# eniac/Reef

Measured on AMD Instinct MI355X. Metric: msm_scalar_point_pairs_per_sec, higher is better.
Workload: dtype u32

## Files before the change

include/reef_msm.h:

```cpp
#ifndef REEF_MSM_H
#define REEF_MSM_H
#define REEF_ABI_VERSION 7

#include <stdbool.h>
#include <stddef.h>
#include <stdint.h>

#ifdef __cplusplus
extern "C" {
#endif

typedef struct { uint64_t l[4]; } reef_fe;
typedef struct { reef_fe x, y; } reef_affine;
typedef struct { reef_fe x, y, z; } reef_jacobian;

enum { REEF_PALLAS = 0, REEF_VESTA = 1 };
enum { REEF_HOST = 0, REEF_DEVICE = 1 };

typedef enum {
    REEF_OK = 0,
    REEF_ERR_ARG = 1,
    REEF_ERR_HIP = 2,
    REEF_ERR_NO_GPU = 3,
    REEF_ERR_OOM = 4
// ... 165 lines not shown
uint32_t reef_abi_version(void);
enum { REEF_WARM_NONE = 0, REEF_WARM_NOW = 1, REEF_WARM_BACKGROUND = 2 };
typedef struct {
    int32_t hw_queues;
    uint32_t warm;
    uint32_t reserved[6];
} reef_runtime_opts;
typedef struct {
    int32_t hw_queues_env;
    int32_t hw_queues_set_by_library;
    uint32_t abi_version;
    uint32_t warm;
} reef_runtime_info;
reef_status reef_runtime_init(const reef_runtime_opts *opts , reef_runtime_info *info );

reef_status reef_msm_ctx_set_window_split(reef_msm_ctx *ctx, uint32_t rank, uint32_t world);
reef_status reef_msm_ctx_enable_timing(reef_msm_ctx *ctx, int on);
reef_status reef_msm_ctx_last_timing(reef_msm_ctx *ctx, float *total_ms, float *accumulate_ms);
reef_status reef_msm_ctx_timing_stats(reef_msm_ctx *ctx, int reset, uint64_t *calls, double *total_ms,
                                      double *accumulate_ms);
reef_status reef_msm_ctx_sum_points(reef_msm_ctx *ctx, const reef_jacobian *in, size_t n, reef_jacobian *out);
reef_status reef_msm_ctx_plan(reef_msm_ctx *ctx, uint32_t *c, uint32_t *windows, uint32_t *groups,
                              uint32_t *tables);

reef_status reef_msm_plan_for(size_t n, uint32_t window_bits, uint32_t bucket_groups, uint32_t *c,
                              uint32_t *windows, uint32_t *groups, uint32_t *tables);

reef_status reef_test_field_op(int field, int op, const reef_fe *a, const reef_fe *b, reef_fe *out, size_t n);
reef_status reef_test_ec_op(int curve, int op, const reef_affine *p, const reef_affine *q, const reef_fe *k,
                            reef_jacobian *out, size_t n);
reef_status reef_bench_fmul(int field, uint32_t iters, double *products_per_s);

typedef struct reef_msm_group reef_msm_group;
enum { REEF_SPLIT_WINDOWS = 0, REEF_SPLIT_POINTS = 1 };
enum { REEF_EXCHANGE_DEFAULT = 0, REEF_EXCHANGE_PEER = 1, REEF_EXCHANGE_HOST = 2, REEF_EXCHANGE_RCCL = 3 };
enum { REEF_SCALARS_EACH = 0, REEF_SCALARS_FANOUT = 1 };
typedef struct {
    uint32_t split;
    uint32_t exchange;
    uint32_t scalars;
    uint32_t reserved[5];
} reef_msm_group_opts;
typedef struct {
    uint32_t members;
    uint32_t distinct_devices;
    uint32_t split, exchange;
// ... 28 lines not shown
```

reef_amd/_ffi.py:

```python
from __future__ import annotations

import ctypes
import os
import subprocess
from ctypes import POINTER, c_bool, c_char_p, c_double, c_float, c_int, c_int32, c_size_t, c_uint8, c_uint32, c_uint64, c_void_p

_HERE = os.path.dirname(os.path.abspath(__file__))
CSRC = os.path.join(_HERE, "csrc")
if os.environ.get("REEF_MSM_HW_QUEUES", "") != "0":
    os.environ.setdefault("GPU_MAX_HW_QUEUES", os.environ.get("REEF_MSM_HW_QUEUES") or "8")
LIB_PATH = os.environ.get("REEF_MSM_LIB") or os.path.join(_HERE, "_lib", "libreef_msm.so")
EXPERIMENT_LIB_PATH = os.path.join(_HERE, "_lib", "libreef_msm_exp.so")
HEADER = os.path.join(os.path.dirname(_HERE), "include", "reef_msm.h")

REEF_HOST, REEF_DEVICE = 0, 1
PALLAS, VESTA = 0, 1
STATUS_NAMES = {0: "REEF_OK", 1: "REEF_ERR_ARG", 2: "REEF_ERR_HIP", 3: "REEF_ERR_NO_GPU", 4: "REEF_ERR_OOM"}


class ReefError(RuntimeError):
    def __init__(self, status: int, message: str):
        super().__init__(f"{STATUS_NAMES.get(status, status)}: {message}")
        self.status = status

# ... 79 lines not shown
        "reef_gen_bases": (c_int, [c_int, c_uint64, c_uint64, c_size_t, vp, c_int]),
        "reef_gen_scalars": (c_int, [c_int, c_uint64, c_int, c_uint64, c_size_t, c_bool, vp, c_int]),
        "reef_device_count": (c_int, []),
        "reef_set_device": (c_int, [c_int]),
        "reef_get_device": (c_int, [POINTER(c_int)]),
        "reef_device_sync": (c_int, []),
        "reef_device_alloc": (vp, [c_size_t]),
        "reef_device_free": (None, [vp]),
        "reef_memcpy": (c_int, [vp, vp, c_size_t, c_int, c_int]),
        "reef_last_error": (c_char_p, []),
        "reef_version": (c_char_p, []),
        "reef_abi_version": (c_uint32, []),
        "reef_key_cache_info": (None, [POINTER(KeyCacheStats)]),
        "reef_key_cache_clear": (None, []),
        "reef_key_cache_wait": (None, []),
        "reef_key_cache_timing_get": (None, [POINTER(KeyCacheTiming), c_int]),
        "reef_runtime_init": (c_int, [POINTER(RuntimeOpts), POINTER(RuntimeInfo)]),
        "reef_msm_ctx_last_timing": (c_int, [vp, POINTER(c_float), POINTER(c_float)]),
        "reef_msm_ctx_enable_timing": (c_int, [vp, c_int]),
        "reef_msm_ctx_set_window_split": (c_int, [vp, c_uint32, c_uint32]),
        "reef_msm_ctx_timing_stats": (c_int, [vp, c_int, POINTER(c_uint64), POINTER(c_double), POINTER(c_double)]),
        "reef_msm_ctx_sum_points": (c_int, [vp, vp, c_size_t, vp]),
        "reef_msm_ctx_plan": (c_int, [vp, POINTER(c_uint32), POINTER(c_uint32), POINTER(c_uint32), POINTER(c_uint32)]),
        "reef_msm_ctx_byte_tables": (c_int, [vp]),
        "reef_msm_plan_for": (c_int, [c_size_t, c_uint32, c_uint32, POINTER(c_uint32), POINTER(c_uint32), POINTER(c_uint32),
                                      POINTER(c_uint32)]),
        "reef_msm_group_create": (c_int, [POINTER(vp), c_int, vp, c_size_t, c_int, POINTER(MsmOpts), POINTER(c_int), c_size_t, POINTER(GroupOpts)]),
        "reef_msm_group_destroy": (None, [vp]),
        "reef_msm_group_info_get": (c_int, [vp, POINTER(GroupInfo)]),
        "reef_msm_group_enable_timing": (c_int, [vp, c_int]),
        "reef_msm_group_last_timing": (c_int, [vp, POINTER(GroupTiming)]),
        "reef_msm_group_msm": (c_int, [vp, vp, c_size_t, c_int, c_bool, vp]),
        "reef_msm_group_rows": (c_int, [vp, vp, c_size_t, c_size_t, c_int, c_bool, c_uint32, vp, vp, vp]),
        "reef_msm_group_rows_symbols": (c_int, [vp, vp, c_size_t, c_size_t, c_int, c_uint32, vp, vp, c_bool, vp]),
        "reef_msm_folded": (c_int, [vp, vp, c_size_t, c_size_t, c_int, c_bool, vp, vp, c_size_t, vp, c_int]),
        "reef_sc_create": (c_int, [POINTER(vp), c_int, c_size_t]),
        "reef_sc_destroy": (None, [vp]),
        "reef_sc_set_table": (c_int, [vp, c_int, vp, c_size_t, c_int]),
        "reef_sc_gen_eq_table": (c_int, [vp, vp, vp, c_size_t, vp, c_size_t]),
        "reef_sc_round_coeffs": (c_int, [vp, c_size_t, vp]),
        "reef_sc_fold": (c_int, [vp, c_size_t, vp]),
        "reef_sc_fold_and_next_coeffs": (c_int, [vp, c_size_t, vp, vp]),
        "reef_sc_read": (c_int, [vp, c_int, c_size_t, vp]),
        "reef_sc_reset_table": (c_int, [vp]),
        "reef_sc_sync": (c_int, [vp]),
        "reef_nifs_create": (c_int, [POINTER(vp), c_int, c_size_t, c_size_t, c_size_t, c_int]),
# ... 95 lines not shown
```

reef_amd/csrc/api.cpp:

```cpp
#include <stdarg.h>
#include <stdio.h>
#include <string>
#include <vector>
#include <new>
#include <exception>
#include <stdlib.h>
#include <string.h>

#include <atomic>
#include <chrono>
#include <condition_variable>
#include <deque>
#include <memory>
#include <mutex>
#include <thread>
#include <type_traits>

#include "common.h"
#include "keccak.h"

namespace reef {

static thread_local char g_err[512] = "";

// ... 264 lines not shown
}
void reef_msm_ctx_destroy(reef_msm_ctx *ctx) { destroy_handle(ctx, &CurveVTable::ctx_destroy); }
reef_status reef_msm_ctx_sync(reef_msm_ctx *ctx) {
    return dispatch<CurveVTable>(ctx, [&](auto *v, void *impl) { return v->ctx_sync(impl); });
}
void *reef_msm_ctx_stream(reef_msm_ctx *ctx) { return ctx ? table<CurveVTable>(ctx->curve)->ctx_stream(ctx->impl) : nullptr; }
reef_status reef_msm_ctx_last_timing(reef_msm_ctx *ctx, float *total_ms, float *accumulate_ms) {
    return dispatch<CurveVTable>(ctx, [&](auto *v, void *impl) { return v->ctx_timing(impl, total_ms, accumulate_ms); });
}
reef_status reef_msm_ctx_set_window_split(reef_msm_ctx *ctx, uint32_t rank, uint32_t world) {
    return dispatch<CurveVTable>(ctx, [&](auto *v, void *impl) { return v->ctx_window_split(impl, rank, world); });
}
reef_status reef_msm_ctx_enable_timing(reef_msm_ctx *ctx, int on) {
    return dispatch<CurveVTable>(ctx, [&](auto *v, void *impl) { return v->ctx_enable_timing(impl, on); });
}
reef_status reef_msm_ctx_timing_stats(reef_msm_ctx *ctx, int reset, uint64_t *calls, double *total_ms, double *accumulate_ms) {
    return dispatch<CurveVTable>(ctx, [&](auto *v, void *impl) { return v->ctx_timing_stats(impl, reset, calls, total_ms, accumulate_ms); });
}
reef_status reef_msm_ctx_sum_points(reef_msm_ctx *ctx, const reef_jacobian *in, size_t n, reef_jacobian *out) {
    return dispatch<CurveVTable>(ctx, [&](auto *v, void *impl) { return v->ctx_sum_points(impl, in, n, out); });
}
reef_status reef_msm_ctx_plan(reef_msm_ctx *ctx, uint32_t *c, uint32_t *windows, uint32_t *groups, uint32_t *tables) {
    return dispatch<CurveVTable>(ctx, [&](auto *v, void *impl) { return v->ctx_plan(impl, c, windows, groups, tables); });
}

reef_status reef_msm(reef_msm_ctx *ctx, const reef_fe *scalars, size_t n, int scalars_loc, bool is_mont, reef_jacobian *out,
                     int out_loc) {
    return dispatch<CurveVTable>(ctx, [&](auto *v, void *impl) { return v->msm(impl, scalars, n, scalars_loc, is_mont, out, out_loc); });
}
reef_status reef_msm_rows(reef_msm_ctx *ctx, const reef_fe *scalars, size_t rows, size_t row_len, int scalars_loc, bool is_mont,
                          uint32_t max_scalar_bits, const reef_fe *blinds, const reef_affine *h, reef_jacobian *out, int out_loc) {
    return dispatch<CurveVTable>(ctx, [&](auto *v, void *impl) { return v->msm_rows(impl, scalars, rows, row_len, scalars_loc, is_mont, max_scalar_bits, blinds, h, out, out_loc); });
}

reef_status reef_msm_multi(size_t count, reef_msm_ctx *const *ctxs, const reef_fe *const *scalars, const size_t *n, int scalars_loc, bool is_mont,
                           reef_jacobian *out) {
    if (count == 0) return REEF_OK;
    if (!ctxs || !scalars || !n || !out || count > 64) { set_error("reef_msm_multi: null argument or more than 64 MSMs"); return REEF_ERR_ARG; }
    for (size_t i = 0; i < count; ++i) {
        if (!ctxs[i]) { set_error("null argument"); return REEF_ERR_ARG; }
        for (size_t j = 0; j < i; ++j)
            if (ctxs[j] == ctxs[i]) { set_error("reef_msm_multi: contexts must be distinct (clone a key that is used twice)"); return REEF_ERR_ARG; }
    }
    static thread_local struct Landing {
        reef_jacobian *p = nullptr;
        ~Landing() { if (p && !g_process_exiting.load()) (void)hipHostFree(p); }
// ... 945 lines not shown
```

reef_amd/csrc/common.h:

```cpp
#pragma once
#include <algorithm>
#include <atomic>
#include <mutex>
#include <thread>
#include <stdio.h>
#include <stdlib.h>
#include <vector>
#include <hip/hip_runtime.h>
#include <stddef.h>
#include <stdint.h>

#include "../../include/reef_msm.h"

namespace reef {

void set_error(const char *fmt, ...) __attribute__((format(printf, 1, 2)));

#define REEF_HIP_TRY(expr)                                                                          \
    do {                                                                                            \
        hipError_t e_ = (expr);                                                                     \
        if (e_ != hipSuccess) {                                                                     \
            ::reef::set_error("%s: %s (%s:%d)", #expr, hipGetErrorString(e_), __FILE__, __LINE__);  \
            return e_ == hipErrorOutOfMemory ? REEF_ERR_OOM : REEF_ERR_HIP;                         \
        }                                                                                           \
// ... 294 lines not shown
struct MerkleSlice {
    uint64_t index_base = 0;
    uint32_t levels = 0;
    const reef_fe *nodes_in = nullptr;
    size_t nodes_n = 0;
    reef_fe *const *level_out = nullptr;
    reef_fe *top_out = nullptr;
};

struct CurveVTable {
    reef_status (*ctx_create)(void **impl, const reef_affine *bases, size_t n, int loc, const reef_msm_opts *opts);
    reef_status (*ctx_rekey)(void *impl, const reef_affine *bases, size_t n, int loc);
    reef_status (*ctx_clone)(void **impl, void *src);
    reef_status (*ctx_attach)(void *impl, void *src_impl);
    void (*ctx_destroy)(void *impl);
    reef_status (*ctx_sync)(void *impl);
    void *(*ctx_stream)(void *impl);
    reef_status (*ctx_timing)(void *impl, float *total_ms, float *acc_ms);
    reef_status (*ctx_enable_timing)(void *impl, int on);
    reef_status (*ctx_window_split)(void *impl, uint32_t rank, uint32_t world);
    reef_status (*ctx_timing_stats)(void *impl, int reset, uint64_t *calls, double *total_ms, double *acc_ms);
    reef_status (*ctx_sum_points)(void *impl, const reef_jacobian *in, size_t n, reef_jacobian *out);
    reef_status (*ctx_plan)(void *impl, uint32_t *c, uint32_t *w, uint32_t *g, uint32_t *t);
    int (*ctx_byte_tables)(void *impl);
    reef_status (*msm)(void *impl, const reef_fe *scalars, size_t n, int loc, bool is_mont, reef_jacobian *out, int out_loc);
    reef_status (*msm_rows)(void *impl, const reef_fe *scalars, size_t rows, size_t row_len, int loc, bool is_mont,
                            uint32_t max_bits, const reef_fe *blinds, const reef_affine *h, reef_jacobian *out, int out_loc);
    reef_status (*msm_rows_symbols)(void *impl, const uint8_t *symbols, size_t rows, size_t row_len, int loc, uint32_t bits,
                                    const reef_fe *blinds, const reef_affine *h, bool blinds_are_mont, reef_jacobian *out, int out_loc);
    reef_status (*ipa_cross)(void *impl, const reef_fe *a, size_t n_k, int loc, bool is_mont, const reef_fe *w1s, const reef_fe *w2s, size_t k,
                             reef_jacobian *out_l, reef_jacobian *out_r);
    reef_status (*msm_folded)(void *impl, const reef_fe *v, size_t len, size_t off, int loc, bool is_mont, const reef_fe *w1s, const reef_fe *w2s,
                              size_t k, reef_jacobian *out, int out_loc);
    reef_status (*fold)(const reef_affine *gens, size_t half, int loc, const reef_fe *w1, const reef_fe *w2, reef_affine *out);
    reef_status (*normalize)(const reef_jacobian *in, size_t n, int loc, reef_affine *out_aff, uint8_t *out_comp);
    reef_status (*sum_points)(const reef_jacobian *in, size_t n, int loc, reef_jacobian *out);
    reef_status (*gen_bases)(uint64_t k0, uint64_t d, size_t n, reef_affine *out, int loc);
    reef_status (*gen_scalars)(uint64_t seed, int kind, uint64_t small_bound, size_t n, bool to_mont, reef_fe *out, int loc);
    reef_status (*test_field_op)(int op, const reef_fe *a, const reef_fe *b, reef_fe *out, size_t n);
    reef_status (*test_ec_op)(int op, const reef_affine *p, const reef_affine *q, const reef_fe *k, reef_jacobian *out, size_t n);
    reef_status (*bench_fmul)(uint32_t iters, double *per_s);
    reef_status (*sc_create)(void **impl, size_t len);
    void (*sc_destroy)(void *impl);
    reef_status (*sc_set)(void *impl, int which, const reef_fe *vals, size_t n, int loc);
    reef_status (*sc_read)(void *impl, int which, size_t count, reef_fe *out_host);
    reef_status (*sc_coeffs)(void *impl, size_t pow, reef_fe *out3_host);
// ... 69 lines not shown
```

reef_amd/csrc/engine.inc:

```
#include <algorithm>
#include <atomic>
#include <mutex>
#include <string.h>
#include <vector>

#include "common.h"
#include "glv_host.h"
#include "host_combine.h"

namespace reef {

static_assert(sizeof(fe256) == sizeof(reef_fe), "fe256 layout");
static_assert(sizeof(affine256) == sizeof(reef_affine), "affine256 layout");
static_assert(sizeof(jacobian256) == sizeof(reef_jacobian), "jacobian256 layout");
static_assert(sizeof(xyzz_mem) == 144, "xyzz_mem layout");

static constexpr u32 MAX_LDS_KEYS = 32768;
static constexpr u32 MAX_SCAN_KEYS = SCAN_TILE * 1024;
static constexpr u32 SORT_SHIFT = 8;
static constexpr u64 TWO_LEVEL_MIN_ENTRIES = 1u << 20;
static constexpr u32 DEFAULT_L0 = 0;

static inline u32 ceil_div(u64 a, u64 b) { return (u32)((a + b - 1) / b); }
static inline u64 round_up(u64 a, u64 b) { return (a + b - 1) / b * b; }
// ... 46 lines not shown
    DevBuf bucket_acc, lkeys[2], lvals[2];
    DevBuf rowcol, group_sums;
    static constexpr int EV_RING = 32;
    hipEvent_t evr[EV_RING][4] = {};
    bool ev_pending[EV_RING] = {};
    int ev_next = 0, ev_last = -1;
    hipEvent_t *ev = nullptr;
    double sum_total_ms = 0, sum_accum_ms = 0;
    u64 timed_calls = 0;
    jacobian256 *pinned = nullptr;
    static constexpr size_t PINNED_POINTS = 64;
    bool timing = false;
    DevBuf sym_table, sym_tmp, sym_u8;
    u32 sym_bits = 0, sym_k = 0, sym_row_len = 0;
    int two_level = -1;
    u32 wsplit_rank = 0, wsplit_world = 1;
    DevBuf h_tab, small_partial;
    DevBuf wide_dig, wide_partial;
    reef_affine h_cached = {};
    const reef_affine *h_host = nullptr;
    bool h_valid = false;
    bool coop = true;
    DevBuf wsum;
    struct GraphEntry {
        const void *scalars; void *out; size_t n; bool is_mont; u32 wr, ww; uint64_t gen; int seen;
        hipGraph_t graph; hipGraphExec_t exec;
    };
    std::vector<GraphEntry> graphs;
};
template <int C> struct CtxScope {
    Ctx<C> *ctx;
    explicit CtxScope(Ctx<C> *c) : ctx(c) {}
    reef_status enter() { return ctx->lease.enter(ctx->key->device, &ctx->stream); }
    ~CtxScope() {
        if (!ctx->lease.counted) return;
        if (hipStreamQuery(ctx->stream) == hipSuccess) ctx->lease.idle();
        else (void)hipGetLastError();
    }
};
template <int C> static void graphs_clear(Ctx<C> *ctx) {
    for (auto &e : ctx->graphs) {
        if (e.exec) (void)hipGraphExecDestroy(e.exec);
        if (e.graph) (void)hipGraphDestroy(e.graph);
    }
    ctx->graphs.clear();
}
// ... 306 lines not shown
    if (G == 1 && n <= SMALL_N_MAX) {
        if (key->small_tab) { (void)hipFree(key->small_tab); key->small_tab = nullptr; }
        REEF_HIP_TRY(hipMalloc((void **)&key->small_tab, small_table_points(n) * sizeof(affine256)));
        REEF_TRY(small_build<C>(ctx, key->tables, n, key->small_tab));
        key->small_n = n;
    }
    REEF_HIP_TRY(hipGetLastError());
    REEF_HIP_TRY(hipStreamSynchronize(ctx->stream));
    if (ctx->tmp_xyzz.cap > (size_t(96) << 20)) ctx->tmp_xyzz.release();
    if (wide_start<C>(key, ctx->opt_tables) != REEF_OK) {
        (void)hipGetLastError();
        wide_drop(key);
    }
    if (ctx->opt_tables == 1) wide_poll<C>(key, true);
    return REEF_OK;
}

template <int C> static void ctx_free(Ctx<C> *ctx) {
    if (!ctx) return;
    graphs_clear(ctx);
    for (DevBuf *b : {&ctx->scalars, &ctx->blinds, &ctx->hpoint, &ctx->dig, &ctx->counts, &ctx->bstart, &ctx->bstart1, &ctx->seg_first,
                      &ctx->seg_counts, &ctx->entries1, &ctx->sym_table, &ctx->sym_tmp, &ctx->sym_u8, &ctx->tile_sums,
                      &ctx->entries, &ctx->bucket_acc, &ctx->rowcol, &ctx->group_sums, &ctx->result,
                      &ctx->tmp_xyzz, &ctx->maxbits, &ctx->wsum, &ctx->h_tab, &ctx->small_partial, &ctx->wide_dig, &ctx->wide_partial, &ctx->lkeys[0], &ctx->lkeys[1], &ctx->lvals[0], &ctx->lvals[1]})
        b->release();
    for (auto &q : ctx->evr)
        for (auto &e : q)
            if (e) (void)hipEventDestroy(e);
    if (ctx->pinned) (void)hipHostFree(ctx->pinned);
    ctx->lease.idle();
    ctx->lease.unpin();
    stream_pool().context_destroyed();
    key_release(ctx->key);
    delete ctx;
}

template <int C> static reef_status ctx_new(Ctx<C> **out, const reef_msm_opts *opts, int *device) {
    REEF_TRY(engine_init_once());
    int dev = -1;
    if (opts && opts->device >= 0) dev = opts->device;
    else REEF_HIP_TRY(hipGetDevice(&dev));
    int ndev = 0;
    REEF_HIP_TRY(hipGetDeviceCount(&ndev));
    if (dev < 0 || dev >= ndev) { set_error("device %d out of range (%d visible)", dev, ndev); return REEF_ERR_ARG; }
    REEF_ON_DEVICE(dev);
    Ctx<C> *ctx = new Ctx<C>();
    if (const char *e = exp_env("REEF_MSM_SORT2")) ctx->two_level = atoi(e);
    if (const char *e = exp_env("REEF_MSM_COOP")) ctx->coop = atoi(e) != 0;
    if (opts) {
        ctx->opt_c = opts->window_bits;
        ctx->opt_G = opts->bucket_groups;
        if (opts->chunk) ctx->L0 = opts->chunk;
        ctx->opt_tables = opts->byte_tables;
    }
    {
        const reef_status st = stream_pool().context_created(dev);
        if (st != REEF_OK) { stream_pool().context_destroyed(); delete ctx; return st; }
    }
    *out = ctx;
    *device = dev;
    return REEF_OK;
}

template <int C>
static reef_status v_ctx_create(void **impl, const reef_affine *bases, size_t n, int loc, const reef_msm_opts *opts) {
    if (!impl || (n && !bases)) { set_error("null argument"); return REEF_ERR_ARG; }
    REEF_TRY(plan_for(n, opts ? opts->window_bits : 0, opts ? opts->bucket_groups : 0, nullptr, nullptr, nullptr, nullptr));
    Ctx<C> *ctx = nullptr;
    int dev = -1;
    REEF_TRY(ctx_new<C>(&ctx, opts, &dev));
    ctx->key = new Key<C>();
// ... 13 lines not shown
template <int C> static reef_status v_ctx_rekey(void *impl, const reef_affine *bases, size_t n, int loc) {
    Ctx<C> *ctx = (Ctx<C> *)impl;
    if (!ctx || (n && !bases)) { set_error("null argument"); return REEF_ERR_ARG; }
    std::lock_guard<std::mutex> lk(ctx->mu);
    if (ctx->key->refs.load() != 1) { set_error("rekey on a shared key"); return REEF_ERR_ARG; }
    REEF_ON_DEVICE(ctx->key->device);
    CtxScope<C> scope(ctx);
    REEF_TRY(scope.enter());
    return key_build<C>(ctx, bases, n, loc);
}

template <int C> static reef_status v_ctx_clone(void **impl, void *src_) {
    Ctx<C> *src = (Ctx<C> *)src_;
    reef_msm_opts o = {};
    o.window_bits = src->opt_c; o.bucket_groups = src->opt_G; o.chunk = src->L0; o.byte_tables = src->opt_tables; o.device = src->key->device;
    Ctx<C> *ctx = nullptr;
    int dev = -1;
    REEF_TRY(ctx_new<C>(&ctx, &o, &dev));
    ctx->key = src->key;
    ++ctx->key->refs;
    ctx->wsplit_rank = src->wsplit_rank;
    ctx->wsplit_world = src->wsplit_world;
    ctx->coop = src->coop;
    *impl = ctx;
    return REEF_OK;
}

template <int C> static reef_status v_ctx_attach(void *impl, void *src_) {
    Ctx<C> *ctx = (Ctx<C> *)impl, *src = (Ctx<C> *)src_;
    if (ctx == src || ctx->key == src->key) return REEF_OK;
    std::lock_guard<std::mutex> lk(ctx->mu);
    if (ctx->key->device != src->key->device) { set_error("attach: the two keys live on different devices"); return REEF_ERR_ARG; }
    REEF_ON_DEVICE(ctx->key->device);
    if (ctx->lease.counted) {
        REEF_HIP_TRY(hipStreamSynchronize(ctx->stream));
        ctx->lease.idle();
    }
    Key<C> *old = ctx->key;
    ctx->key = src->key;
    ++ctx->key->refs;
    key_release(old);
    ctx->opt_c = src->opt_c; ctx->opt_G = src->opt_G; ctx->opt_tables = src->opt_tables;
    ctx->wsplit_rank = src->wsplit_rank;
    ctx->wsplit_world = src->wsplit_world;
    ctx->sym_bits = 0;
    graphs_clear(ctx);
// ... 59 lines not shown
    return REEF_OK;
}
template <int C> static reef_status v_ctx_timing_stats(void *impl, int reset, uint64_t *calls, double *total_ms, double *acc_ms) {
    Ctx<C> *ctx = (Ctx<C> *)impl;
    std::lock_guard<std::mutex> lk(ctx->mu);
    for (int i = 0; i < Ctx<C>::EV_RING; ++i) REEF_TRY(ctx_harvest<C>(ctx, i));
    if (calls) *calls = ctx->timed_calls;
    if (total_ms) *total_ms = ctx->sum_total_ms;
    if (acc_ms) *acc_ms = ctx->sum_accum_ms;
    if (reset) { ctx->timed_calls = 0; ctx->sum_total_ms = ctx->sum_accum_ms = 0; }
    return REEF_OK;
}
template <int C> static reef_status v_ctx_sum_points(void *impl, const reef_jacobian *in, size_t n, reef_jacobian *out) {
    Ctx<C> *ctx = (Ctx<C> *)impl;
    if (!in || !out || n > 65536) { set_error("bad argument"); return REEF_ERR_ARG; }
    std::lock_guard<std::mutex> lk(ctx->mu);
    REEF_ON_DEVICE(ctx->key->device);
    CtxScope<C> scope(ctx);
    REEF_TRY(scope.enter());
    hipLaunchKernelGGL(k_sum_points<C>, dim3(1), dim3(64), 0, ctx->stream, (const jacobian256 *)in, (u32)n, (jacobian256 *)out);
    REEF_HIP_TRY(hipGetLastError());
    return REEF_OK;
}
template <int C> static reef_status v_ctx_plan(void *impl, uint32_t *c, uint32_t *w, uint32_t *g, uint32_t *t) {
    Key<C> *k = ((Ctx<C> *)impl)->key;
    if (c) *c = k->c;
    if (w) *w = k->W;
    if (g) *g = k->G;
    if (t) *t = k->T;
    return REEF_OK;
}

struct CorePlan {
    u32 c, W, G;
    u32 rows, row_len;
    u32 n_ctx;
    bool slice_sort = false;
};

template <int C> static bool merge_is_fused(const Ctx<C> *ctx, u32 nchunks0) {
    static const bool on = !(exp_env("REEF_MSM_FUSE_MERGE") && atoi(exp_env("REEF_MSM_FUSE_MERGE")) == 0);
    static const bool merge1 = !(exp_env("REEF_MSM_MERGE1") && atoi(exp_env("REEF_MSM_MERGE1")) == 0);
    static const u32 max_chunks = [] { const char *e = exp_env("REEF_MSM_FUSE_MAX_CHUNKS"); return e ? (u32)atoi(e) : 65536u; }();
    const u32 waves = ceil_div(nchunks0, 64);
    return on && merge1 && nchunks0 <= max_chunks && !(ctx->coop && waves <= 384);
}
template <int C>
static void launch_partial_merge(Ctx<C> *ctx, u32 nchunks0, xyzz_mem *acc, bool first_level_done = false) {
    hipStream_t st = ctx->stream;
    u32 waves = ceil_div(nchunks0, 64);
    static const bool merge1 = !(exp_env("REEF_MSM_MERGE1") && atoi(exp_env("REEF_MSM_MERGE1")) == 0);
    u32 len = 2 * waves;
// ... 182 lines not shown
        const void *ent = (const void *)ctx->entries.template as<u32x2>();
        xyzz_mem *bacc = ctx->bucket_acc.template as<xyzz_mem>();
        u32 *ok = ctx->lkeys[fused ? 1 : 0].template as<u32>();
        xyzz_mem *ov = ctx->lvals[fused ? 1 : 0].template as<xyzz_mem>();
        if (fused && word_entries) hipLaunchKernelGGL((k_accum0<C, true, true>), ag, ab, 0, st, ctx->key->tables, ent, bstart + NBT, L0, nchunks0, bacc, ok, ov, NBT);
        else if (fused) hipLaunchKernelGGL((k_accum0<C, true, false>), ag, ab, 0, st, ctx->key->tables, ent, bstart + NBT, L0, nchunks0, bacc, ok, ov, 0u);
        else if (word_entries) hipLaunchKernelGGL((k_accum0<C, false, true>), ag, ab, 0, st, ctx->key->tables, ent, bstart + NBT, L0, nchunks0, bacc, ok, ov, NBT);
        else hipLaunchKernelGGL((k_accum0<C, false, false>), ag, ab, 0, st, ctx->key->tables, ent, bstart + NBT, L0, nchunks0, bacc, ok, ov, 0u);
    }
    if (ctx->timing) REEF_HIP_TRY(hipEventRecord(ctx->ev[2], st));
    launch_partial_merge<C>(ctx, nchunks0, ctx->bucket_acc.template as<xyzz_mem>(), fused);

    const u32 lg = pl.c - 1;
    const u32 c2 = (lg + 1) / 2, c1 = lg - c2;
    const u32 per_group = (1u << c1) + (1u << c2);
    const u32 rc_waves = groups_total * per_group;
    xyzz_mem *gsum = ctx->group_sums.template as<xyzz_mem>();
    if (group_sums_out && ctx->pinned && (size_t)groups_total * sizeof(xyzz_mem) <= Ctx<C>::PINNED_POINTS * sizeof(jacobian256))
        gsum = (xyzz_mem *)ctx->pinned;
    const bool direct = !group_sums_out && pl.G == 1;
    static const int skip_reduce = [] { const char *e = exp_env("REEF_MSM_SKIP_REDUCE"); return e ? atoi(e) : 0; }();
    if (skip_reduce == 1) {
        if (group_sums_out) *group_sums_out = gsum;
    } else if (ctx->coop) {
        REEF_TRY(ctx->wsum.ensure((u64)groups_total * 4 * sizeof(xyzz_mem)));
        if (skip_reduce != 2)
        hipLaunchKernelGGL(k_reduce_rowcol_coop<C>, dim3(rc_waves), dim3(256), 0, st, ctx->bucket_acc.template as<xyzz_mem>(), bstart, c1, c2,
                           groups_total, ctx->rowcol.template as<xyzz_mem>());
        hipLaunchKernelGGL(k_reduce_weighted_coop<C>, dim3(groups_total, 2), dim3(256), 0, st, ctx->rowcol.template as<xyzz_mem>(), c1, c2,
                           ctx->wsum.template as<xyzz_mem>());
        hipLaunchKernelGGL(k_reduce_combine_coop<C>, dim3(groups_total), dim3(256), 0, st, ctx->wsum.template as<xyzz_mem>(), c2, gsum,
                           direct ? d_out : (jacobian256 *)nullptr);
    } else {
        if (skip_reduce != 2)
        hipLaunchKernelGGL(k_reduce_rowcol<C>, dim3(ceil_div(rc_waves, 4)), dim3(256), 0, st, ctx->bucket_acc.template as<xyzz_mem>(),
                           bstart, c1, c2, groups_total, ctx->rowcol.template as<xyzz_mem>());
        hipLaunchKernelGGL(k_reduce_weighted<C>, dim3(groups_total), dim3(128), 0, st, ctx->rowcol.template as<xyzz_mem>(), c1, c2, gsum,
                           direct ? d_out : (jacobian256 *)nullptr);
    }
    const xyzz_mem *gs = gsum;
    if (skip_reduce == 1) {}
    else if (group_sums_out) *group_sums_out = gs;
    else if (!direct) hipLaunchKernelGGL(k_final<C>, dim3(ceil_div(pl.rows, 64)), dim3(64), 0, st, gs, pl.G, pl.c, pl.rows, d_out);
    if (d_blinds && (ctx->wsplit_world <= 1 || ctx->wsplit_rank == 0))
        REEF_TRY(launch_blind<C>(ctx, d_out, d_blinds, d_h, is_mont, pl.rows));
    if (ctx->timing) {
        REEF_HIP_TRY(hipEventRecord(ctx->ev[3], st));
        ctx->ev_pending[ctx->ev_last] = true;
    }
    REEF_HIP_TRY(hipGetLastError());
    return REEF_OK;
}

template <int C>
static reef_status result_target(Ctx<C> *ctx, size_t count, reef_jacobian *out, int out_loc, jacobian256 **d_res) {
    if (out_loc == REEF_DEVICE) { *d_res = (jacobian256 *)out; return REEF_OK; }
    if (count <= Ctx<C>::PINNED_POINTS) {
        if (!ctx->pinned) REEF_HIP_TRY(hipHostMalloc((void **)&ctx->pinned, Ctx<C>::PINNED_POINTS * sizeof(jacobian256), hipHostMallocDefault));
        *d_res = ctx->pinned;
        return REEF_OK;
    }
// ... 843 lines not shown
        u32 pick = 0;
        for (u32 d = 0; d <= 18 && !pick; ++d) {
            if (cc >= 2 + d && fits(cc - d)) pick = cc - d;
            else if (cc + d <= 20 && fits(cc + d)) pick = cc + d;
        }
        if (!pick) { set_error("no window size fits a key of %zu points with bucket_groups = %u", n, g_opt); return REEF_ERR_ARG; }
        cc = pick;
    } else if (!fits(cc)) {
        set_error("window_bits = %u with bucket_groups = %u needs %llu bucket keys / %llu digits for %zu points (limits: %u keys, 2^32 digits)",
                  cc, g_opt, (unsigned long long)((u64)groups_of(cc) << (cc - 1)), (unsigned long long)((u64)n * windows_for(cc)), n, MAX_SCAN_KEYS);
        return REEF_ERR_ARG;
    }
    const u32 W = windows_for(cc);
    const u32 G = groups_of(cc);
    if (c) *c = cc;
    if (w) *w = W;
    if (g) *g = G;
    if (t) *t = ceil_div(W, G);
    return REEF_OK;
}

template <int C> static CurveVTable make_vtable() {
    return CurveVTable{v_ctx_create<C>, v_ctx_rekey<C>, v_ctx_clone<C>, v_ctx_attach<C>, v_ctx_destroy<C>, v_ctx_sync<C>, v_ctx_stream<C>,
                       v_ctx_timing<C>, v_ctx_enable_timing<C>, v_ctx_window_split<C>, v_ctx_timing_stats<C>, v_ctx_sum_points<C>, v_ctx_plan<C>, v_ctx_byte_tables<C>, v_msm<C>, v_msm_rows<C>, v_msm_rows_symbols<C>, v_ipa_cross<C>, v_msm_folded<C>, v_fold<C>, v_normalize<C>, v_sum_points<C>,
                       v_gen_bases<C>, v_gen_scalars<C>, v_test_field_op<C>, v_test_ec_op<C>, v_bench_fmul<C>,
                       v_sc_create<C>, v_sc_destroy<C>, v_sc_set<C>, v_sc_read<C>, v_sc_coeffs<C>, v_sc_fold<C>, v_sc_fold_coeffs<C>, v_sc_gen_eq<C>, v_sc_reset<C>, v_sc_sync<C>, v_mle_bound<C>, v_merkle_commit<C>, v_derive_generators<C>, plan_for};
}

}
```

reef_amd/csrc/msm_kernels.inc:

```
#include "ec.h"
#include "ec_coop.h"
#include "glv_consts.h"

namespace reef {

static constexpr u32 KEY_INVALID = 0xffffffffu;
static constexpr int WAVE = 64;

template <int C> struct Kern;

__device__ __forceinline__ void latency_critical() { __builtin_amdgcn_s_setprio(3); }

__device__ __forceinline__ u32 extract_bits(const fe256 &k, u32 off, u32 c) {
    const u32 limb = off >> 5, sh = off & 31u;
    u32 lo = 0, hi = 0;
#pragma unroll
    for (u32 l = 0; l < 8; ++l) {
        lo = (l == limb) ? k.w[l] : lo;
        hi = (l == limb + 1) ? k.w[l] : hi;
    }
    u64 v = (((u64)hi << 32) | lo) >> sh;
    return (u32)v & ((1u << c) - 1u);
}

// ... 960 lines not shown
        bool take;
        if (step < nload) {
            const u32 e = step * 64u + lane;
            const u32 key = first + e * stride;
            take = e < count && bucket_start[key + 1] != bucket_start[key];
            if (take) o = load_xyzz_coop(bucket_acc + key);
        } else {
            const int d = 32 >> (step - nload);
            const bool o_live = __shfl(live ? 1 : 0, (lane + d) & 63, WAVE) != 0;
            take = lane < d && o_live;
            if (__any(take)) o = shfl_xyzz(acc, (lane + d) & 63);
        }
        if (__any(take)) {
            if (__any(take && live)) {
                const xyzz sum = xyzz_add_coop<C>(acc, o, L, role, lane);
                acc = xyzz_select(take, live ? sum : o, acc);
            } else {
                acc = xyzz_select(take, o, acc);
            }
            live = live || take;
        }
    }
    if (threadIdx.x == 0) store_xyzz(rowcol + (size_t)g * per_group + idx, acc);
}

template <int C>
__device__ __forceinline__ void coop_weighted_sum(const xyzz_mem *__restrict__ in, u32 count, int lane, int role, CoopLds &L, xyzz &X, xyzz &T) {
    const u32 s = count >= 64 ? count / 64 : 1;
    const u32 lanes = count >= 64 ? 64 : count;
    const bool has = (u32)lane < lanes;
    const u32 e0 = (u32)lane * s;
    xyzz R = xyzz_identity(), A = xyzz_identity();
    if (has) R = load_xyzz_coop(in + e0 + s - 1);
    if (s > 1) A = R;
    enum { RUN_R, RUN_A, SCAN, SHIFT, JOIN, TREE, DONE };
    int phase = s > 1 ? RUN_R : SCAN;
    int t = (int)s - 2;
    int d = 1;
    u32 k = 1;
    T = xyzz_identity();
    for (;;) {
        if (phase == SCAN && (u32)d >= lanes) { T = R; phase = s > 1 ? SHIFT : JOIN; }
        if (phase == SHIFT && k >= s) phase = JOIN;
        if (phase == JOIN && lanes <= 1) phase = TREE, d = 32;
        if (phase == JOIN && s == 1) {
            A = xyzz_select(lane >= 1, R, A);
// ... 1087 lines not shown
```

reef_amd/msm.py:

```python
from __future__ import annotations

import ctypes
from typing import Optional, Tuple, Union

import numpy as np

from . import _ffi
from ._fe import _Handle
from ._ffi import PALLAS, REEF_DEVICE, REEF_HOST, VESTA, MsmOpts, ReefError, check

CURVE_IDS = {"pallas": PALLAS, "vesta": VESTA, PALLAS: PALLAS, VESTA: VESTA}
PALLAS_BASE_P = 0x40000000000000000000000000000000224698fc094cf91b992d30ed00000001
PALLAS_SCALAR_Q = 0x40000000000000000000000000000000224698fc0994a8dd8c46eb2100000001
SCALAR_MODULUS = {PALLAS: PALLAS_SCALAR_Q, VESTA: PALLAS_BASE_P}
Buf = Union[np.ndarray, "DeviceBuffer", int]


def curve_id(curve) -> int:
    try:
        return CURVE_IDS[curve]
    except KeyError:
        raise ValueError(f"unknown curve {curve!r}") from None


# ... 82 lines not shown
        self.n = n

    def clone(self) -> "MsmContext":
        h = ctypes.c_void_p()
        check(self._lib.reef_msm_ctx_clone(ctypes.byref(h), self._h))
        return MsmContext(self.curve, None, self.n, _handle=h)

    def attach(self, other: "MsmContext") -> None:
        check(self._lib.reef_msm_ctx_attach(self._h, other._h))
        self.n = other.n

    def sync(self) -> None:
        check(self._lib.reef_msm_ctx_sync(self._h))

    @property
    def stream(self) -> int:
        return self._lib.reef_msm_ctx_stream(self._h) or 0

    def plan(self) -> dict:
        c, w, g, t = (ctypes.c_uint32() for _ in range(4))
        check(self._lib.reef_msm_ctx_plan(self._h, ctypes.byref(c), ctypes.byref(w), ctypes.byref(g), ctypes.byref(t)))
        return {"window_bits": c.value, "windows": w.value, "bucket_groups": g.value, "tables": t.value}

    def has_byte_tables(self) -> bool:
        return bool(self._lib.reef_msm_ctx_byte_tables(self._h))

    def set_window_split(self, rank: int, world: int) -> None:
        check(self._lib.reef_msm_ctx_set_window_split(self._h, rank, world))

    def enable_timing(self, on: bool = True) -> None:
        check(self._lib.reef_msm_ctx_enable_timing(self._h, int(on)))

    def last_timing(self) -> Tuple[float, float]:
        a, b = ctypes.c_float(), ctypes.c_float()
        check(self._lib.reef_msm_ctx_last_timing(self._h, ctypes.byref(a), ctypes.byref(b)))
        return a.value, b.value

    def timing_stats(self, reset: bool = True) -> dict:
        calls, tot, acc = ctypes.c_uint64(), ctypes.c_double(), ctypes.c_double()
        check(self._lib.reef_msm_ctx_timing_stats(self._h, int(reset), ctypes.byref(calls), ctypes.byref(tot), ctypes.byref(acc)))
        return {"calls": calls.value, "total_ms": tot.value, "accumulate_ms": acc.value}

    def sum_points(self, jac: Buf, n: int, out: Buf) -> Buf:
        loc, ptr = _loc_ptr(jac, 96 * n)
        oloc, optr = _loc_ptr(out, 96)
        if loc != REEF_DEVICE or oloc != REEF_DEVICE:
# ... 261 lines not shown
```

Measured before the change: 901.9 million.

## Add multi-stage per-lane segmented row/column bucket reduction for large MSMs

Adds a new row/column reduction path in which each thread sums a segment of 8 buckets, repeated in stages until each row and column is reduced to one point. This replaces the cooperative wave-per-line kernel when the window is wide or n is large. It spreads the reduction across many more independent lanes to raise occupancy, at the cost of extra launches and intermediate partial buffers. The choice is made by a heuristic, can be overridden by an environment variable, and is exposed through a new API query.

```diff
diff --git a/include/reef_msm.h b/include/reef_msm.h
--- a/include/reef_msm.h
+++ b/include/reef_msm.h
@@ -211,6 +211,7 @@
 reef_status reef_msm_ctx_sum_points(reef_msm_ctx *ctx, const reef_jacobian *in, size_t n, reef_jacobian *out);
 reef_status reef_msm_ctx_plan(reef_msm_ctx *ctx, uint32_t *c, uint32_t *windows, uint32_t *groups,
                               uint32_t *tables);
+reef_status reef_msm_ctx_reduce_form(reef_msm_ctx *ctx, size_t n, uint32_t *lanes);
 
 reef_status reef_msm_plan_for(size_t n, uint32_t window_bits, uint32_t bucket_groups, uint32_t *c,
                               uint32_t *windows, uint32_t *groups, uint32_t *tables);
diff --git a/reef_amd/_ffi.py b/reef_amd/_ffi.py
--- a/reef_amd/_ffi.py
+++ b/reef_amd/_ffi.py
@@ -125,6 +125,7 @@
         "reef_msm_ctx_timing_stats": (c_int, [vp, c_int, POINTER(c_uint64), POINTER(c_double), POINTER(c_double)]),
         "reef_msm_ctx_sum_points": (c_int, [vp, vp, c_size_t, vp]),
         "reef_msm_ctx_plan": (c_int, [vp, POINTER(c_uint32), POINTER(c_uint32), POINTER(c_uint32), POINTER(c_uint32)]),
+        "reef_msm_ctx_reduce_form": (c_int, [vp, c_size_t, POINTER(c_uint32)]),
         "reef_msm_ctx_byte_tables": (c_int, [vp]),
         "reef_msm_plan_for": (c_int, [c_size_t, c_uint32, c_uint32, POINTER(c_uint32), POINTER(c_uint32), POINTER(c_uint32),
                                       POINTER(c_uint32)]),
diff --git a/reef_amd/csrc/api.cpp b/reef_amd/csrc/api.cpp
--- a/reef_amd/csrc/api.cpp
+++ b/reef_amd/csrc/api.cpp
@@ -310,6 +310,9 @@
 }
 reef_status reef_msm_ctx_plan(reef_msm_ctx *ctx, uint32_t *c, uint32_t *windows, uint32_t *groups, uint32_t *tables) {
     return dispatch<CurveVTable>(ctx, [&](auto *v, void *impl) { return v->ctx_plan(impl, c, windows, groups, tables); });
+}
+reef_status reef_msm_ctx_reduce_form(reef_msm_ctx *ctx, size_t n, uint32_t *lanes) {
+    return dispatch<CurveVTable>(ctx, [&](auto *v, void *impl) { return v->ctx_reduce_form(impl, n, lanes); });
 }
 
 reef_status reef_msm(reef_msm_ctx *ctx, const reef_fe *scalars, size_t n, int scalars_loc, bool is_mont, reef_jacobian *out,
diff --git a/reef_amd/csrc/common.h b/reef_amd/csrc/common.h
--- a/reef_amd/csrc/common.h
+++ b/reef_amd/csrc/common.h
@@ -340,6 +340,7 @@
     reef_status (*ctx_timing_stats)(void *impl, int reset, uint64_t *calls, double *total_ms, double *acc_ms);
     reef_status (*ctx_sum_points)(void *impl, const reef_jacobian *in, size_t n, reef_jacobian *out);
     reef_status (*ctx_plan)(void *impl, uint32_t *c, uint32_t *w, uint32_t *g, uint32_t *t);
+    reef_status (*ctx_reduce_form)(void *impl, size_t n, uint32_t *lanes);
     int (*ctx_byte_tables)(void *impl);
     reef_status (*msm)(void *impl, const reef_fe *scalars, size_t n, int loc, bool is_mont, reef_jacobian *out, int out_loc);
     reef_status (*msm_rows)(void *impl, const reef_fe *scalars, size_t rows, size_t row_len, int loc, bool is_mont,
diff --git a/reef_amd/csrc/engine.inc b/reef_amd/csrc/engine.inc
--- a/reef_amd/csrc/engine.inc
+++ b/reef_amd/csrc/engine.inc
@@ -92,6 +92,8 @@
     bool h_valid = false;
     bool coop = true;
     DevBuf wsum;
+    int reduce_lanes = -1;
+    DevBuf rc_part;
     struct GraphEntry {
         const void *scalars; void *out; size_t n; bool is_mont; u32 wr, ww; uint64_t gen; int seen;
         hipGraph_t graph; hipGraphExec_t exec;
@@ -444,7 +446,7 @@
     for (DevBuf *b : {&ctx->scalars, &ctx->blinds, &ctx->hpoint, &ctx->dig, &ctx->counts, &ctx->bstart, &ctx->bstart1, &ctx->seg_first,
                       &ctx->seg_counts, &ctx->entries1, &ctx->sym_table, &ctx->sym_tmp, &ctx->sym_u8, &ctx->tile_sums,
                       &ctx->entries, &ctx->bucket_acc, &ctx->rowcol, &ctx->group_sums, &ctx->result,
-                      &ctx->tmp_xyzz, &ctx->maxbits, &ctx->wsum, &ctx->h_tab, &ctx->small_partial, &ctx->wide_dig, &ctx->wide_partial, &ctx->lkeys[0], &ctx->lkeys[1], &ctx->lvals[0], &ctx->lvals[1]})
+                      &ctx->tmp_xyzz, &ctx->maxbits, &ctx->wsum, &ctx->rc_part, &ctx->h_tab, &ctx->small_partial, &ctx->wide_dig, &ctx->wide_partial, &ctx->lkeys[0], &ctx->lkeys[1], &ctx->lvals[0], &ctx->lvals[1]})
         b->release();
     for (auto &q : ctx->evr)
         for (auto &e : q)
@@ -469,6 +471,7 @@
     Ctx<C> *ctx = new Ctx<C>();
     if (const char *e = exp_env("REEF_MSM_SORT2")) ctx->two_level = atoi(e);
     if (const char *e = exp_env("REEF_MSM_COOP")) ctx->coop = atoi(e) != 0;
+    if (const char *e = exp_env("REEF_MSM_REDUCE_LANES")) ctx->reduce_lanes = atoi(e) != 0;
     if (opts) {
         ctx->opt_c = opts->window_bits;
         ctx->opt_G = opts->bucket_groups;
@@ -528,6 +531,7 @@
     ctx->wsplit_rank = src->wsplit_rank;
     ctx->wsplit_world = src->wsplit_world;
     ctx->coop = src->coop;
+    ctx->reduce_lanes = src->reduce_lanes;
     *impl = ctx;
     return REEF_OK;
 }
@@ -633,12 +637,47 @@
     REEF_HIP_TRY(hipGetLastError());
     return REEF_OK;
 }
+static constexpr u32 REDUCE_LANES_MIN_LG = 15, REDUCE_LANES_MIN_TOTAL_LG = 19, REDUCE_LANES_MIN_POINTS_LG = 20;
+template <int C> static bool reduce_uses_lanes(const Ctx<C> *ctx, u32 c, u64 groups, u64 n) {
+    if (ctx->reduce_lanes >= 0) return ctx->reduce_lanes != 0;
+    if (c - 1 < REDUCE_LANES_MIN_LG) return false;
+    return (groups << (c - 1)) >= (1ull << REDUCE_LANES_MIN_TOTAL_LG) || n >= (1ull << REDUCE_LANES_MIN_POINTS_LG);
+}
+template <int C>
+static reef_status launch_rowcol_lanes(Ctx<C> *ctx, hipStream_t st, const u32 *bstart, u32 c1, u32 c2, u32 groups_total) {
+    const u64 rows = 1ull << c1, cols = 1ull << c2;
+    auto partials = [&](u64 nr, u64 nc) { return groups_total * (rows * ceil_div(nr, (u64)REDUCE_SEG) + cols * ceil_div(nc, (u64)REDUCE_SEG)); };
+    const u64 size_a = partials(cols, rows);
+    const u64 size_b = partials(ceil_div(cols, (u64)REDUCE_SEG), ceil_div(rows, (u64)REDUCE_SEG));
+    REEF_TRY(ctx->rc_part.ensure((size_a + size_b) * sizeof(xyzz_mem)));
+    xyzz_mem *region[2] = {ctx->rc_part.template as<xyzz_mem>(), ctx->rc_part.template as<xyzz_mem>() + size_a};
+    const xyzz_mem *in = region[1];
+    u32 nr = (u32)cols, nc = (u32)rows;
+    for (int stage = 0;; ++stage) {
+        const u32 pr = ceil_div(nr, REDUCE_SEG), pc = ceil_div(nc, REDUCE_SEG);
+        const bool last = pr == 1 && pc == 1;
+        xyzz_mem *out = last ? ctx->rowcol.template as<xyzz_mem>() : region[stage & 1];
+        const u32 lanes = (u32)partials(nr, nc);
+        hipLaunchKernelGGL(k_reduce_rowcol_lanes<C>, dim3(ceil_div(lanes, 64u)), dim3(64), 0, st, ctx->bucket_acc.template as<xyzz_mem>(), bstart,
+                           in, c1, c2, groups_total, nr, nc, (int)(stage == 0), out);
+        if (last) break;
+        in = out; nr = pr; nc = pc;
+    }
+    return REEF_OK;
+}
+
 template <int C> static reef_status v_ctx_plan(void *impl, uint32_t *c, uint32_t *w, uint32_t *g, uint32_t *t) {
     Key<C> *k = ((Ctx<C> *)impl)->key;
     if (c) *c = k->c;
     if (w) *w = k->W;
     if (g) *g = k->G;
     if (t) *t = k->T;
+    return REEF_OK;
+}
+template <int C> static reef_status v_ctx_reduce_form(void *impl, size_t n, uint32_t *lanes) {
+    Ctx<C> *ctx = (Ctx<C> *)impl;
+    if (!lanes) { set_error("null argument"); return REEF_ERR_ARG; }
+    *lanes = reduce_uses_lanes<C>(ctx, ctx->key->c, ctx->key->G, n) ? 1u : 0u;
     return REEF_OK;
 }
 
@@ -867,21 +906,24 @@
     static const int skip_reduce = [] { const char *e = exp_env("REEF_MSM_SKIP_REDUCE"); return e ? atoi(e) : 0; }();
     if (skip_reduce == 1) {
         if (group_sums_out) *group_sums_out = gsum;
-    } else if (ctx->coop) {
-        REEF_TRY(ctx->wsum.ensure((u64)groups_total * 4 * sizeof(xyzz_mem)));
-        if (skip_reduce != 2)
-        hipLaunchKernelGGL(k_reduce_rowcol_coop<C>, dim3(rc_waves), dim3(256), 0, st, ctx->bucket_acc.template as<xyzz_mem>(), bstart, c1, c2,
-                           groups_total, ctx->rowcol.template as<xyzz_mem>());
-        hipLaunchKernelGGL(k_reduce_weighted_coop<C>, dim3(groups_total, 2), dim3(256), 0, st, ctx->rowcol.template as<xyzz_mem>(), c1, c2,
-                           ctx->wsum.template as<xyzz_mem>());
-        hipLaunchKernelGGL(k_reduce_combine_coop<C>, dim3(groups_total), dim3(256), 0, st, ctx->wsum.template as<xyzz_mem>(), c2, gsum,
-                           direct ? d_out : (jacobian256 *)nullptr);
     } else {
-        if (skip_reduce != 2)
-        hipLaunchKernelGGL(k_reduce_rowcol<C>, dim3(ceil_div(rc_waves, 4)), dim3(256), 0, st, ctx->bucket_acc.template as<xyzz_mem>(),
-                           bstart, c1, c2, groups_total, ctx->rowcol.template as<xyzz_mem>());
-        hipLaunchKernelGGL(k_reduce_weighted<C>, dim3(groups_total), dim3(128), 0, st, ctx->rowcol.template as<xyzz_mem>(), c1, c2, gsum,
-                           direct ? d_out : (jacobian256 *)nullptr);
+        xyzz_mem *bacc = ctx->bucket_acc.template as<xyzz_mem>(), *rowcol = ctx->rowcol.template as<xyzz_mem>();
+        if (skip_reduce == 2) {
+        } else if (reduce_uses_lanes<C>(ctx, pl.c, groups_total, N)) {
+            REEF_TRY(launch_rowcol_lanes<C>(ctx, st, bstart, c1, c2, groups_total));
+        } else if (ctx->coop) {
+            hipLaunchKernelGGL(k_reduce_rowcol_coop<C>, dim3(rc_waves), dim3(256), 0, st, bacc, bstart, c1, c2, groups_total, rowcol);
+        } else {
+            hipLaunchKernelGGL(k_reduce_rowcol<C>, dim3(ceil_div(rc_waves, 4)), dim3(256), 0, st, bacc, bstart, c1, c2, groups_total, rowcol);
+        }
+        if (ctx->coop) {
+            REEF_TRY(ctx->wsum.ensure((u64)groups_total * 4 * sizeof(xyzz_mem)));
+            hipLaunchKernelGGL(k_reduce_weighted_coop<C>, dim3(groups_total, 2), dim3(256), 0, st, rowcol, c1, c2, ctx->wsum.template as<xyzz_mem>());
+            hipLaunchKernelGGL(k_reduce_combine_coop<C>, dim3(groups_total), dim3(256), 0, st, ctx->wsum.template as<xyzz_mem>(), c2, gsum,
+                               direct ? d_out : (jacobian256 *)nullptr);
+        } else {
+            hipLaunchKernelGGL(k_reduce_weighted<C>, dim3(groups_total), dim3(128), 0, st, rowcol, c1, c2, gsum, direct ? d_out : (jacobian256 *)nullptr);
+        }
     }
     const xyzz_mem *gs = gsum;
     if (skip_reduce == 1) {}
@@ -1771,7 +1813,7 @@
 
 template <int C> static CurveVTable make_vtable() {
     return CurveVTable{v_ctx_create<C>, v_ctx_rekey<C>, v_ctx_clone<C>, v_ctx_attach<C>, v_ctx_destroy<C>, v_ctx_sync<C>, v_ctx_stream<C>,
-                       v_ctx_timing<C>, v_ctx_enable_timing<C>, v_ctx_window_split<C>, v_ctx_timing_stats<C>, v_ctx_sum_points<C>, v_ctx_plan<C>, v_ctx_byte_tables<C>, v_msm<C>, v_msm_rows<C>, v_msm_rows_symbols<C>, v_ipa_cross<C>, v_msm_folded<C>, v_fold<C>, v_normalize<C>, v_sum_points<C>,
+                       v_ctx_timing<C>, v_ctx_enable_timing<C>, v_ctx_window_split<C>, v_ctx_timing_stats<C>, v_ctx_sum_points<C>, v_ctx_plan<C>, v_ctx_reduce_form<C>, v_ctx_byte_tables<C>, v_msm<C>, v_msm_rows<C>, v_msm_rows_symbols<C>, v_ipa_cross<C>, v_msm_folded<C>, v_fold<C>, v_normalize<C>, v_sum_points<C>,
                        v_gen_bases<C>, v_gen_scalars<C>, v_test_field_op<C>, v_test_ec_op<C>, v_bench_fmul<C>,
                        v_sc_create<C>, v_sc_destroy<C>, v_sc_set<C>, v_sc_read<C>, v_sc_coeffs<C>, v_sc_fold<C>, v_sc_fold_coeffs<C>, v_sc_gen_eq<C>, v_sc_reset<C>, v_sc_sync<C>, v_mle_bound<C>, v_merkle_commit<C>, v_derive_generators<C>, plan_for};
 }
diff --git a/reef_amd/csrc/msm_kernels.inc b/reef_amd/csrc/msm_kernels.inc
--- a/reef_amd/csrc/msm_kernels.inc
+++ b/reef_amd/csrc/msm_kernels.inc
@@ -1006,6 +1006,52 @@
         }
     }
     if (threadIdx.x == 0) store_xyzz(rowcol + (size_t)g * per_group + idx, acc);
+}
+
+static constexpr u32 REDUCE_SEG = 8;
+template <int C>
+__global__ void __launch_bounds__(64) k_reduce_rowcol_lanes(const xyzz_mem *__restrict__ bucket_acc, const u32 *__restrict__ bucket_start,
+                                                           const xyzz_mem *__restrict__ in, u32 c1, u32 c2, u32 groups, u32 nr, u32 nc,
+                                                           int first, xyzz_mem *__restrict__ out) {
+    latency_critical();
+    const u32 rows = 1u << c1, cols = 1u << c2;
+    const u32 pr = (nr + REDUCE_SEG - 1u) / REDUCE_SEG, pc = (nc + REDUCE_SEG - 1u) / REDUCE_SEG;
+    const u32 per_in = rows * nr + cols * nc, per_out = rows * pr + cols * pc;
+    const u32 t = blockIdx.x * blockDim.x + threadIdx.x;
+    if (t >= groups * per_out) return;
+    const u32 g = t / per_out, r = t - g * per_out;
+    const bool is_row = r < rows * pr;
+    u32 line, seg;
+    if (is_row) { line = r / pr; seg = r - line * pr; }
+    else { const u32 q = r - rows * pr; seg = q >> c2; line = q & (cols - 1u); }
+    const u32 count = is_row ? nr : nc;
+    const u32 e0 = seg * REDUCE_SEG;
+    const u32 key0 = (g << (c1 + c2)) + (is_row ? line << c2 : line);
+    const xyzz_mem *line_in = in + (size_t)g * per_in + (is_row ? line * nr : rows * nr + line * nc);
+    xyzz acc = xyzz_identity();
+    bool live = false;
+#pragma unroll 1
+    for (u32 k = 0; k < REDUCE_SEG; ++k) {
+        const u32 e = e0 + k;
+        bool take = e < count;
+        const xyzz_mem *src = line_in + e;
+        if (first) {
+            const u32 key = key0 + (is_row ? e : e << c2);
+            take = take && bucket_start[key + 1] != bucket_start[key];
+            src = bucket_acc + key;
+        }
+        if (!__any(take)) continue;
+        xyzz b = xyzz_identity();
+        if (take) b = load_xyzz(src);
+        if (__any(take && live)) {
+            const xyzz s = xyzz_add<C>(acc, b);
+            acc = xyzz_select(take, live ? s : b, acc);
+        } else {
+            acc = xyzz_select(take, b, acc);
+        }
+        live = live || take;
+    }
+    store_xyzz(out + (size_t)g * per_out + (is_row ? line * pr + seg : rows * pr + line * pc + seg), acc);
 }
 
 template <int C>
diff --git a/reef_amd/msm.py b/reef_amd/msm.py
--- a/reef_amd/msm.py
+++ b/reef_amd/msm.py
@@ -128,6 +128,11 @@
         check(self._lib.reef_msm_ctx_plan(self._h, ctypes.byref(c), ctypes.byref(w), ctypes.byref(g), ctypes.byref(t)))
         return {"window_bits": c.value, "windows": w.value, "bucket_groups": g.value, "tables": t.value}
 
+    def reduce_form(self, n: Optional[int] = None) -> str:
+        lanes = ctypes.c_uint32()
+        check(self._lib.reef_msm_ctx_reduce_form(self._h, self.n if n is None else n, ctypes.byref(lanes)))
+        return "lanes" if lanes.value else "coop"
+
     def has_byte_tables(self) -> bool:
         return bool(self._lib.reef_msm_ctx_byte_tables(self._h))
 
```

Result: faster. 920.5 million, median of 6 (+2.1%).
